# vsahni3/cross-attention-ViT

Measured on AMD Instinct MI355X. Metric: 3D patch-tokens/sec fwd+bwd, 2-modality 128^3 p16 ViT, higher is better.
Workload: dtype bf16; 1 GPU; configs[1]: ModelCross d=768 H=12 mlp=3072 2x2 blocks, 2 modalities, 128^3 volume, 16^3 patches (N=513), dropout 0; per_gpu_batch=126, global_batch=126, seq_len=513, parallelism=dp1, step=zero-grad + weight bf16 cast + fwd + loss + bwd, optimizer_step=excluded, launch=eager (one launch per kernel)

## Files before the change

cross-attention-vit_amd/csrc/gemm.hip:

```cpp
#include "xvit_common.h"

#include <atomic>
#include <algorithm>
#include <string>

namespace xvit {

struct GemmParams {
  const bf16* A = nullptr; const bf16* B = nullptr; void* C = nullptr; const float* bias = nullptr; const float* res = nullptr; bf16* aux = nullptr;
  int64_t lda = 0, ldb = 0, ldc = 0, ldr = 0, ldaux = 0;
  int64_t sA = 0, sB = 0, sC = 0, sBias = 0, sR = 0, sAux = 0;
  int M = 0, N = 0, K = 0, k_per_split = 0, split_k = 1, ntm = 0, ntn = 0;
  int c_f32 = 0, act = XVIT_ACT_NONE, accumulate = 0;
  int res_row_mod = 0, res_row_off = 0, seg_rows = 0, seg_skip = 0, row_off = 0;
  float* slab = nullptr;
  float* colsum = nullptr;
  float drop_p = 0.f, drop_inv = 1.f; uint64_t drop_seed = 0;
  const uint64_t* drop_epoch = nullptr;
  int aux_deriv = 0;
  int narrow_epi = 0;
  int ncg = 1;
  struct PatchGather {
    int mode = 0;
    int dp, hp, wp;
    int Dn, Wn;
    int Sy, Sz;
    int pcount, ntok, cls;
    int nb;
    int64_t sBt, sMd;
    uint32_t vol_bytes;
    uint32_t m_pcount, m_dn, m_wn, m_nb;
    uint32_t m_ntok;
  } g;
};

constexpr uint32_t GATHER_OOB = 0x80000000u;
constexpr uint32_t OOB = 0xFFFFFFF0u;
typedef __attribute__((__vector_size__(2 * sizeof(unsigned)))) unsigned u32x2_t;
// ... 234 lines not shown
      for (int kk = 0; kk < 2; ++kk) off[kk] = (uint32_t)(row * 128 + (((kk * 4 + (lane >> 4)) ^ swz_kc(row)) << 4));
    }
  }
  __device__ __forceinline__ bf16x8 read(const XVIT_LDS char* image, int t, int kk) const {
#ifdef XVIT_DEBUG_NO_LDSREAD
    if constexpr (W == 256) {
      u32x4_t v = {off[0] * 2654435761u, off[0] * 40503u + 12345u, (uint32_t)t * 0x9E3779B9u ^ off[0], 0x3F803F80u ^ (off[0] << 3)};
      v &= 0xBFFFBFFFu;
      asm volatile("" : "+v"(v));
      return __builtin_bit_cast(bf16x8, v);
    }
#endif
    if (KS) {
      const s16x4 lo = lds_read_tr16(image + off[t * 2 + 0] + kk * 32 * PITCH);
      const s16x4 hi = lds_read_tr16(image + off[t * 2 + 1] + kk * 32 * PITCH);
      s16x8 v = {lo[0], lo[1], lo[2], lo[3], hi[0], hi[1], hi[2], hi[3]};
      return __builtin_bit_cast(bf16x8, v);
    } else {
      return *(const XVIT_LDS bf16x8*)(image + off[kk] + t * 16 * 128);
    }
  }
};

template <bool A_KS, bool B_KS>
__global__ __launch_bounds__(256, 2) void gemm_kernel(const GemmParams p) {
  extern __shared__ __attribute__((aligned(16))) char smem_raw[];
  XVIT_LDS char* smem = (XVIT_LDS char*)smem_raw;
  const int tid = threadIdx.x, lane = tid & 63, wave = uniform(tid >> 6);
  const int wr = wave >> 1, wc = wave & 1;

  const int logical = xcd_logical(blockIdx.x, gridDim.x);
  const int tm = logical / p.ntn, tn = logical - tm * p.ntn;
  const int m0 = tm * BM, n0 = tn * BN;
  const int batch = blockIdx.z / p.split_k, split = blockIdx.z - batch * p.split_k;
  const int k_begin = split * p.k_per_split;
  const int k_end = min(p.K, k_begin + p.k_per_split);
  const int nk = (k_end - k_begin + BK - 1) / BK;
  TileLoader<A_KS, BM> la;
  TileLoader<B_KS, BN> lb;
  la.init(operand_tile<A_KS>(p.A + batch * p.sA, p.lda, m0, p.M, k_begin, k_end), p.lda, wave, lane);
  lb.init(operand_tile<B_KS>(p.B + batch * p.sB, p.ldb, n0, p.N, k_begin, k_end), p.ldb, wave, lane);
  TileFrag<A_KS, BM, 4> fa;
  TileFrag<B_KS, BN, 4> fb;
  fa.init(wr * 4, lane);
  fb.init(wc * 4, lane);

  f32x4 acc[4][4];
// ... 48 lines not shown
#pragma unroll
    for (int mi = 0; mi < 2; ++mi)
#pragma unroll
      for (int j = 0; j < 4; ++j)
#pragma unroll
        for (int r = 0; r < 4; ++r)
          slab[(mi * 16 + (lane >> 4) * 4 + r) * EPI_LD + j * 16 + (lane & 15)] = acc[pass * 2 + mi][j][r];
    const int row_base = m0 + wr * 64 + pass * 32;
#pragma unroll 1
    for (int it = 0; it < 8; ++it) {
      const int rl = it * 4 + (lane >> 4);
      const int row = row_base + rl;
      const f32x4 v = *(const XVIT_LDS f32x4*)(slab + rl * EPI_LD + (lane & 15) * 4);
      if (row < p.M && col < p.N) {
        if (part) {
          *(f32x4*)(part + (int64_t)row * p.N + col) = v;
        } else {
          cs4 += epilogue_apply_rt(p, v, row, col, cb, bias, res, aux);
        }
      }
    }
  }
  if (csum && !part) colsum_flush<16>(csum + col, cs4, col < p.N);
}

constexpr int TBM = 256, TBN = 256;
constexpr int T_OPER = TBM * BK * 2;
constexpr int T_STAGE = 2 * T_OPER;
constexpr int T_LDS = 2 * T_STAGE;

__device__ __forceinline__ uint32_t gather_soff_rows(const GemmParams::PatchGather& g, int ktg) { return 2u * gather_elem_off(g, ktg * 64); }
struct GatherStep { uint32_t a, b; };
__device__ __forceinline__ GatherStep gather_soff_wgrad(const GemmParams::PatchGather& g, int ktg, int64_t lda) {
  const int spk = g.pcount >> 6, smp = ktg / spk, r = ktg - smp * spk;
  const int wsteps = (g.Dn * g.Wn) >> 6, h = r / wsteps, wpart = (r - h * wsteps) * (64 / g.Dn);
  GatherStep o;
  o.a = (uint32_t)(((int64_t)smp * g.ntok + g.cls + r * 64) * lda * 2);
  o.b = 2u * (gather_sample_origin(g, smp) + (uint32_t)(h * g.hp * g.Sy + wpart * g.wp));
  return o;
}

template <int S, int PF, int NA, int NB>
__device__ __forceinline__ void mma_sched_steps() {
  constexpr int reads = (S + PF < 16 ? NA : 0) + (S >= 4 && S < 8 ? NB : 0);
  if constexpr (reads > 0) __builtin_amdgcn_sched_group_barrier(0x100, reads, 0);
  __builtin_amdgcn_sched_group_barrier(0x008, 4, 0);
// ... 381 lines not shown
  const int wl = pin_lane(lane);
  Transpose8 t;
  t.init(wl);
  ScatterEpi e;
  e.vol = (char*)p.C;
  const uint32_t col = (uint32_t)(col0 + (wl & 7) * 8);
  e.col_ok = col < (uint32_t)p.N;
  e.eoff = e.col_ok ? gather_elem_off(p.g, (int)col) : 0u;
  e.row = (uint32_t)(row0 + (wl >> 3));
  struct NoLoads {} none;
  transpose8_regions<0>(t, acc, smem + wave * EPI_WAVE_BYTES, none, [](NoLoads&) {}, [&](f32x4 v0, f32x4 v1, const NoLoads&, int) { scatter_body(p, e, v0, v1); });
}

#ifdef XVIT_GEMM_CLOCK_PROBE
__device__ long long xvit_dbg_clk[2 * 4096];
struct ClockProbe {
  long long c0, w0;
  __device__ ClockProbe() : c0(clock64()), w0(wall_clock64()) {}
  __device__ ~ClockProbe() {
    if (threadIdx.x == 0 && blockIdx.z == 0 && blockIdx.x < 4096) { xvit_dbg_clk[2 * blockIdx.x] = clock64() - c0; xvit_dbg_clk[2 * blockIdx.x + 1] = wall_clock64() - w0; }
  }
};
#endif
template <bool A_KS, bool B_KS, int WIDE_ACT, int GATHER = 0>
__global__ __launch_bounds__(512, 2) void gemm_big_kernel(const GemmParams p) {
  extern __shared__ __attribute__((aligned(16))) char smem_raw[];
  XVIT_LDS char* smem = (XVIT_LDS char*)smem_raw;
#ifdef XVIT_GEMM_CLOCK_PROBE
  ClockProbe clock_probe;
#endif
  const int tid = threadIdx.x, lane = tid & 63, wave = uniform(tid >> 6);
  const int wr = wave >> 2, wc = wave & 3;

  const int nblk = gridDim.x;
  const int logical = xcd_logical(blockIdx.x + nblk * blockIdx.z, nblk * gridDim.z);
  const int zz = logical / nblk, tile = logical - zz * nblk;
  const int grp = min(tile / (p.ntm * p.ncg), (p.ntn - 1) / p.ncg);
  const int rem = tile - grp * p.ntm * p.ncg;
  const int gw = min(p.ncg, p.ntn - grp * p.ncg);
  const int tm = rem / gw, tn = grp * p.ncg + (rem - tm * gw);
  const int m0 = tm * TBM, n0 = tn * TBN;
  const int batch = zz / p.split_k, split = zz - batch * p.split_k;
  const int k_begin = split * p.k_per_split;
  const int k_end = min(p.K, k_begin + p.k_per_split);
  const int nk = (k_end - k_begin + BK - 1) / BK;

  TileLoader<A_KS, TBM> la;
// ... 41 lines not shown
    uint32_t oa, ob;
    step_off(0, oa, ob);
    la.issue_at(smem, wave, oa);
    lb.issue_at(smem + T_OPER, wave, ob);
  }
  for (int kt = 0; kt < nk; ++kt) {
    asm volatile("s_waitcnt vmcnt(0)" ::: "memory");
    __syncthreads();
    const bool more = kt + 1 < nk;
    uint32_t soff_a, soff_b;
    step_off(kt + 1, soff_a, soff_b);
    XVIT_LDS char* nxt = smem + ((kt + 1) & 1) * T_STAGE;
    const XVIT_LDS char* sa = smem + (kt & 1) * T_STAGE;
    const XVIT_LDS char* sb = sa + T_OPER;
#ifndef XVIT_DEBUG_NO_MMA
    big_tile_mma<A_KS, B_KS>(sa, sb, fa, fb, acc, la, lb, more ? la.rsrc : null_rsrc, more ? lb.rsrc : null_rsrc, nxt, wave, soff_a, soff_b);
#endif
  }

  asm volatile("s_waitcnt vmcnt(0)" ::: "memory");
  __syncthreads();
  if constexpr (GATHER == 4) scatter_epilogue(p, acc, smem, wave, lane, m0 + wr * 128, n0 + wc * 64);
  else if constexpr (WIDE_ACT >= 0) wave_tile_epilogue_wide<WIDE_ACT>(p, acc, smem, wave, lane, m0 + wr * 128, n0 + wc * 64, batch);
  else wave_tile_epilogue<GATHER == 1>(p, acc, smem, wave, lane, m0 + wr * 128, n0 + wc * 64, batch, split);
}

__global__ void splitk_epilogue_kernel(const GemmParams p, int nbatch) {
  const int nv = p.N >> 2;
  const int64_t per = (int64_t)p.M * nv, total = per * nbatch;
  for (int64_t i = (int64_t)blockIdx.x * blockDim.x + threadIdx.x; i < total; i += (int64_t)gridDim.x * blockDim.x) {
    const int b = (int)(i / per);
    const int64_t r = i - (int64_t)b * per;
    const int row = (int)(r / nv), col = (int)(r - (int64_t)row * nv) * 4;
    f32x4 v = {0.f, 0.f, 0.f, 0.f};
    for (int s = 0; s < p.split_k; ++s) v += *(const f32x4*)(p.slab + (((int64_t)s * nbatch + b) * p.M + row) * p.N + col);
    const f32x4 o = epilogue_apply_rt(p, v, row, col, b * p.sC, p.bias ? p.bias + b * p.sBias : nullptr, p.res ? p.res + b * p.sR : nullptr,
                                      p.aux ? p.aux + b * p.sAux : nullptr);
    if (p.colsum) {
#pragma unroll
      for (int e = 0; e < 4; ++e) unsafeAtomicAdd(p.colsum + b * p.sBias + col + e, o[e]);
    }
  }
}

}

using namespace xvit;

static bool aligned16(const void* p) { return (reinterpret_cast<uintptr_t>(p) & 15) == 0; }

static std::atomic<int> g_gemm_tile{0};
static std::atomic<int> g_gemm_epi{0};
static std::atomic<int> g_gemm_group{0};

static bool use_big_tile(const xvit_gemm_args* a) {
  if (a->M < 256 || a->N < 256 || g_gemm_tile.load(std::memory_order_relaxed) == 1) return false;
  if (g_gemm_tile.load(std::memory_order_relaxed) == 2) return true;
  const int64_t big_blocks = (int64_t)((a->M + 255) / 256) * ((a->N + 255) / 256) * a->batch * (a->split_k > 0 ? a->split_k : 1);
  return big_blocks > 128;
}

static int k_per_split(int K, int split_k) {
  const int ktiles = (K + BK - 1) / BK;
  return ((ktiles + split_k - 1) / split_k) * BK;
}

static void set_tile_grid(GemmParams& p, int tile, int layout, bool grouped = true) {
  p.ntm = (p.M + tile - 1) / tile; p.ntn = (p.N + tile - 1) / tile;
  p.ncg = p.ntn;
  if (grouped) {
    const int forced = g_gemm_group.load(std::memory_order_relaxed);
    p.ncg = forced > 0 ? std::min(forced, p.ntn) : (layout == XVIT_GEMM_NT && p.ntn >= 6 ? 3 : p.ntn);
  }
}

template <bool A_KS, bool B_KS, int WIDE_ACT, int GATHER = 0>
static void launch_big(const GemmParams& p, int grid_z, hipStream_t s) {
  launch_lds<gemm_big_kernel<A_KS, B_KS, WIDE_ACT, GATHER>, T_LDS, 512>(dim3(p.ntm * p.ntn, 1, grid_z), s, p);
}
template <bool A_KS, bool B_KS>
static void launch_small(const GemmParams& p, int grid_z, hipStream_t s) {
  launch_lds<gemm_kernel<A_KS, B_KS>, GEMM_LDS, 256>(dim3(p.ntm * p.ntn, 1, grid_z), s, p);
}
static void launch_splitk_reduce(const GemmParams& p, int nbatch, hipStream_t s) {
  const int64_t work = (int64_t)nbatch * p.M * (p.N / 4);
  const int g = (int)((work + 255) / 256 > 4096 ? 4096 : (work + 255) / 256);
  hipLaunchKernelGGL(splitk_epilogue_kernel, dim3(g), dim3(256), 0, s, p, nbatch);
}

extern "C" int xvit_set_option(const char* name, int value) {
  XVIT_REQUIRE(name != nullptr, "xvit_set_option: null name");
  const std::string n(name);
  if (n == "gemm_tile") { XVIT_REQUIRE(value >= 0 && value <= 2, "xvit_set_option: gemm_tile must be 0 (auto), 1 (128x128 only) or 2 (256x256 whenever M, N >= 256)"); g_gemm_tile = value; return 0; }
  if (n == "gemm_group") { XVIT_REQUIRE(value >= 0 && value <= 4096, "xvit_set_option: gemm_group must be in [0, 4096]"); g_gemm_group = value; return 0; }
  if (n == "gemm_epilogue") { XVIT_REQUIRE(value == 0 || value == 1, "xvit_set_option: gemm_epilogue must be 0 (auto) or 1 (narrow)"); g_gemm_epi = value; return 0; }
  if (n == "attn_peel") { XVIT_REQUIRE(value >= 0 && value <= 2, "xvit_set_option: attn_peel must be 0 (token 0 stays on the tile grid), 1 (auto: large grids) or 2 (whenever N = 64 m + 1)"); set_attn_peel(value); return 0; }
  set_error("xvit_set_option: unknown option '%s'", name);
  return XVIT_ERR_ARG;
}

extern "C" int64_t xvit_gemm_workspace_bytes(const xvit_gemm_args* a) {
  if (!a || a->split_k <= 1) return 0;
  return (int64_t)a->split_k * a->batch * a->M * a->N * (int64_t)sizeof(float);
}

extern "C" int xvit_gemm(const xvit_gemm_args* a, xvit_stream_t stream) {
  XVIT_REQUIRE(a != nullptr, "xvit_gemm: null args");
  XVIT_REQUIRE(a->layout >= 0 && a->layout <= 2, "xvit_gemm: bad layout %d", a->layout);
  XVIT_REQUIRE(a->M > 0 && a->N > 0 && a->K > 0 && a->batch > 0, "xvit_gemm: M,N,K,batch must be > 0 (got %d,%d,%d,%d)", a->M, a->N, a->K, a->batch);
  XVIT_REQUIRE(a->A && a->B && a->C, "xvit_gemm: null A/B/C");
  const bool a_ks = a->layout == XVIT_GEMM_TN, b_ks = a->layout != XVIT_GEMM_NT;
  XVIT_REQUIRE(a_ks || a->K % 64 == 0, "xvit_gemm: K=%d must be a multiple of 64 when A is k-contiguous", a->K);
  XVIT_REQUIRE(b_ks || a->K % 64 == 0, "xvit_gemm: K=%d must be a multiple of 64 when B is k-contiguous", a->K);
  XVIT_REQUIRE(a->N % 4 == 0, "xvit_gemm: N=%d must be a multiple of 4 (use xvit_small_linear_*)", a->N);
  XVIT_REQUIRE(a->lda % 8 == 0 && a->ldb % 8 == 0 && a->stride_a % 8 == 0 && a->stride_b % 8 == 0, "xvit_gemm: lda/ldb/strides must be multiples of 8 elements");
  XVIT_REQUIRE(aligned16(a->A) && aligned16(a->B) && aligned16(a->C), "xvit_gemm: A/B/C must be 16-byte aligned");
  XVIT_REQUIRE(a->ldc % 4 == 0 && a->stride_c % 4 == 0, "xvit_gemm: ldc/stride_c must be multiples of 4");
  XVIT_REQUIRE(a->lda >= (a_ks ? a->M : a->K) && a->ldb >= (b_ks ? a->N : a->K) && a->ldc >= a->N, "xvit_gemm: leading dimension smaller than the row length");
  const int64_t a_rows = a_ks ? a->K : a->M, b_rows = b_ks ? a->K : a->N;
  XVIT_REQUIRE(a_rows * a->lda * 2 < (1ll << 31) && b_rows * a->ldb * 2 < (1ll << 31), "xvit_gemm: an operand matrix exceeds 2 GiB (unsupported addressing range)");
  XVIT_REQUIRE(a->split_k >= 1, "xvit_gemm: split_k must be >= 1");
  {
// ... 16 lines not shown
                 a->split_k, (long long)ws_need, (long long)a->workspace_bytes);

  GemmParams p;
  p.A = (const bf16*)a->A; p.B = (const bf16*)a->B; p.C = a->C; p.bias = a->bias; p.res = a->residual; p.aux = (bf16*)a->aux;
  p.lda = a->lda; p.ldb = a->ldb; p.ldc = a->ldc; p.ldr = a->ldr; p.ldaux = a->ldaux;
  p.sA = a->stride_a; p.sB = a->stride_b; p.sC = a->stride_c; p.sBias = a->stride_bias; p.sR = a->stride_r; p.sAux = a->stride_aux;
  p.M = a->M; p.N = a->N; p.K = a->K; p.split_k = a->split_k;
  p.k_per_split = k_per_split(a->K, a->split_k);
  p.c_f32 = a->c_dtype == XVIT_F32; p.act = a->act; p.accumulate = a->accumulate;
  p.res_row_mod = a->res_row_mod; p.res_row_off = a->res_row_off;
  p.seg_rows = a->out_seg_rows; p.seg_skip = a->out_seg_skip; p.row_off = a->out_row_off;
  p.slab = ws_need > 0 ? (float*)a->workspace : nullptr;
  p.colsum = a->colsum;
  XVIT_REQUIRE(a->dropout_p >= 0.f && a->dropout_p < 1.f, "xvit_gemm: dropout_p must be in [0, 1)");
  p.drop_p = a->dropout_p; p.drop_inv = 1.0f / (1.0f - a->dropout_p); p.drop_seed = a->dropout_seed;
  p.drop_epoch = a->dropout_p > 0.f ? drop_epoch_ptr() : nullptr;
  p.narrow_epi = g_gemm_epi.load(std::memory_order_relaxed);
  p.aux_deriv = a->aux_mode;
  hipStream_t s = (hipStream_t)stream;
  const int gz = a->batch * a->split_k;

  if (big) {
    set_tile_grid(p, TBM, a->layout);
    const bool wide = !p.c_f32 && !p.slab && !p.res && p.seg_rows == 0 && !p.narrow_epi && p.drop_p == 0.f && a->layout != XVIT_GEMM_TN &&
                      ((p.N | (int)p.ldc | (int)p.ldaux) & 7) == 0 && (a->layout == XVIT_GEMM_NT ? p.act != XVIT_ACT_DGELU : p.act != XVIT_ACT_GELU);
    if (wide && a->layout == XVIT_GEMM_NT && p.act == XVIT_ACT_NONE) launch_big<false, false, XVIT_ACT_NONE>(p, gz, s);
    else if (wide && a->layout == XVIT_GEMM_NT && p.aux_deriv) launch_big<false, false, ACT_GELU_D>(p, gz, s);
    else if (wide && a->layout == XVIT_GEMM_NT) launch_big<false, false, XVIT_ACT_GELU>(p, gz, s);
    else if (wide && p.act == XVIT_ACT_NONE) launch_big<false, true, XVIT_ACT_NONE>(p, gz, s);
    else if (wide && p.aux_deriv) launch_big<false, true, ACT_MULAUX>(p, gz, s);
    else if (wide) launch_big<false, true, XVIT_ACT_DGELU>(p, gz, s);
    else if (a->layout == XVIT_GEMM_NT) launch_big<false, false, -1>(p, gz, s);
    else if (a->layout == XVIT_GEMM_NN) launch_big<false, true, -1>(p, gz, s);
    else launch_big<true, true, -1>(p, gz, s);
  } else {
    set_tile_grid(p, BM, a->layout, false);
    switch (a->layout) {
      case XVIT_GEMM_NT: launch_small<false, false>(p, gz, s); break;
      case XVIT_GEMM_NN: launch_small<false, true>(p, gz, s); break;
      default: launch_small<true, true>(p, gz, s); break;
    }
  }
  if (p.slab) launch_splitk_reduce(p, a->batch, s);
  return check_launch("xvit_gemm");
}

static int64_t pe_rows(const xvit_patch_geom* g) {
  return (int64_t)g->M * g->B * (g->cls_rows + (int64_t)(g->D / g->dp) * (g->H / g->hp) * (g->W / g->wp));
}

static bool pe_geom_ok(const xvit_patch_geom* g) {
  if (!g || g->B <= 0 || g->M <= 0 || g->dp <= 0 || g->hp <= 0 || g->wp <= 0 || (g->cls_rows != 0 && g->cls_rows != 1)) return false;
  return !(g->D % g->dp || g->H % g->hp || g->W % g->wp);
}

extern "C" int xvit_patch_embed_supported(const xvit_patch_geom* g, int d) {
  if (!pe_geom_ok(g)) return 0;
  const int Dn = g->D / g->dp, Hn = g->H / g->hp, Wn = g->W / g->wp;
  const int64_t pd = (int64_t)g->dp * g->hp * g->wp, pcount = (int64_t)Dn * Hn * Wn;
  if (g->wp % 8 || 64 % g->wp || (g->hp * g->wp) % 64) return 0;
  if (pd % 256 || d % 256 || d < 256) return 0;
  const int64_t rows = pe_rows(g);
  if (rows < 2048) return 0;
  if ((int64_t)g->B * g->M * g->D * g->H * g->W * 2 >= (1ll << 31)) return 0;
  if (rows * d * 4 >= (1ll << 31) || pcount > (1 << 24)) return 0;
  return 1;
// ... 62 lines not shown
                                      int64_t workspace_bytes, xvit_stream_t stream) {
  XVIT_REQUIRE(img && g && dx && dW, "xvit_patch_embed_wgrad: null pointer");
  XVIT_REQUIRE(xvit_patch_embed_supported(g, d) == 1, "xvit_patch_embed_wgrad: geometry not supported by the fused kernel (xvit_patch_embed_supported)");
  const int64_t pd = (int64_t)g->dp * g->hp * g->wp;
  XVIT_REQUIRE(lddx >= d && lddx % 8 == 0 && lddw >= pd && lddw % 4 == 0, "xvit_patch_embed_wgrad: bad leading dimension");
  XVIT_REQUIRE(aligned16(img) && aligned16(dx) && aligned16(dW), "xvit_patch_embed_wgrad: pointers must be 16-byte aligned");
  XVIT_REQUIRE(pe_rows(g) * lddx * 2 < (1ll << 31), "xvit_patch_embed_wgrad: dx exceeds 2 GiB (unsupported addressing range)");
  const int64_t need = xvit_patch_embed_wgrad_workspace_bytes(g, d);
  XVIT_REQUIRE(need == 0 || (workspace && workspace_bytes >= need && aligned16(workspace)), "xvit_patch_embed_wgrad: needs %lld bytes of 16-byte aligned workspace (got %lld)",
               (long long)need, (long long)workspace_bytes);
  GemmParams p;
  pe_defaults(p);
  const bool aligned = pe_aligned(g);
  pe_fill(p, g, aligned ? 2 : 3);
  p.A = (const bf16*)dx; p.B = (const bf16*)img; p.C = dW;
  p.lda = lddx; p.ldc = lddw;
  p.M = d; p.N = (int)pd;
  p.K = (int)((int64_t)g->M * g->B * p.g.pcount);
  p.split_k = pe_wgrad_split(g, d);
  p.k_per_split = k_per_split(p.K, p.split_k);
  p.slab = need > 0 ? (float*)workspace : nullptr;
  set_tile_grid(p, TBM, XVIT_GEMM_TN, false);
  hipStream_t s = (hipStream_t)stream;
  if (aligned) launch_big<true, true, -1, 2>(p, p.split_k, s);
  else launch_big<true, true, -1, 3>(p, p.split_k, s);
  if (p.slab) launch_splitk_reduce(p, 1, s);
  return check_launch("xvit_patch_embed_wgrad");
}

extern "C" int xvit_patch_embed_dgrad_supported(const xvit_patch_geom* g, int d) {
  if (!pe_geom_ok(g)) return 0;
  if (g->wp % 8) return 0;
  if (d % 64 || d < 64) return 0;
  const int64_t rows = pe_rows(g);
  if (rows < 2048) return 0;
  if ((int64_t)g->B * g->M * g->D * g->H * g->W >= (1ll << 30)) return 0;
  if (rows * d * 2 >= (1ll << 31)) return 0;
  if ((int64_t)(g->D / g->dp) * (g->H / g->hp) * (g->W / g->wp) > (1 << 24)) return 0;
  return 1;
}

extern "C" int xvit_patch_embed_dgrad(const void* dx, int64_t lddx, const void* W, int64_t ldw, const xvit_patch_geom* g, int d, void* dimg, int dimg_dtype,
                                      xvit_stream_t stream) {
  XVIT_REQUIRE(dx && W && g && dimg, "xvit_patch_embed_dgrad: null pointer");
  XVIT_REQUIRE(dimg_dtype == XVIT_F32 || dimg_dtype == XVIT_BF16, "xvit_patch_embed_dgrad: bad output dtype %d", dimg_dtype);
  XVIT_REQUIRE(xvit_patch_embed_dgrad_supported(g, d) == 1, "xvit_patch_embed_dgrad: geometry not supported by the fused kernel (xvit_patch_embed_dgrad_supported)");
  const int64_t pd = (int64_t)g->dp * g->hp * g->wp;
  XVIT_REQUIRE(lddx >= d && lddx % 8 == 0 && ldw >= pd && ldw % 8 == 0, "xvit_patch_embed_dgrad: bad leading dimension");
  XVIT_REQUIRE(aligned16(dx) && aligned16(W) && aligned16(dimg), "xvit_patch_embed_dgrad: pointers must be 16-byte aligned");
// ... 18 lines not shown
```

cross-attention-vit_amd/csrc/linear_f32.hip:

```cpp
#include "xvit_common.h"

namespace xvit {

struct F32Params {
  const float* A; const float* W; float* C; const float* bias; const float* res; float* slab;
  bf16* c_bf16; bf16* z_bf16;
  int64_t lda, ldw, ldc, ldr, ldcb, ldzb;
  int M, N, K, k_per_split, split_k, act;
  Dropout drop;
};

__device__ __forceinline__ void f32_epilogue(const F32Params& p, float v, int row, int col) {
  if (p.bias) v += p.bias[col];
  if (p.act == XVIT_ACT_GELU) {
    if (p.z_bf16) p.z_bf16[(int64_t)row * p.ldzb + col] = f2bf(v);
    v = gelu_f(v);
  }
  if (p.drop.on()) v = p.drop.at_run_time().keep((uint64_t)row * p.N + col) ? v * p.drop.inv : 0.f;
  if (p.res) v += p.res[(int64_t)row * p.ldr + col];
  p.C[(int64_t)row * p.ldc + col] = v;
  if (p.c_bf16) p.c_bf16[(int64_t)row * p.ldcb + col] = f2bf(v);
}

__global__ __launch_bounds__(64) void linear_f32_kernel(const F32Params p) {
  const int lane = threadIdx.x, r = lane & 31, h = lane >> 5;
  const int ntn = (p.N + 31) >> 5;
  const int tm = blockIdx.x / ntn, tn = blockIdx.x - tm * ntn, split = blockIdx.y;
  const int m0 = tm * 32, n0 = tn * 32;
  const int kb = split * p.k_per_split, ke = min(p.K, kb + p.k_per_split);
  const float* ap = p.A + (int64_t)min(m0 + r, p.M - 1) * p.lda + 4 * h;
  const float* wp = p.W + (int64_t)min(n0 + r, p.N - 1) * p.ldw + 4 * h;
  f32x16 acc;
#pragma unroll
  for (int i = 0; i < 16; ++i) acc[i] = 0.f;
#pragma unroll 2
  for (int k = kb; k < ke; k += 16) {
    const f32x4 a0 = *(const f32x4*)(ap + k), a1 = *(const f32x4*)(ap + k + 8);
    const f32x4 w0 = *(const f32x4*)(wp + k), w1 = *(const f32x4*)(wp + k + 8);
#pragma unroll
    for (int e = 0; e < 4; ++e) acc = __builtin_amdgcn_mfma_f32_32x32x2f32(a0[e], w0[e], acc, 0, 0, 0);
#pragma unroll
    for (int e = 0; e < 4; ++e) acc = __builtin_amdgcn_mfma_f32_32x32x2f32(a1[e], w1[e], acc, 0, 0, 0);
  }
  const int col = n0 + r;
  if (col >= p.N) return;
#pragma unroll
  for (int t = 0; t < 16; ++t) {
    const int row = m0 + acc_row(t, h);
    if (row < p.M) {
      if (p.slab) p.slab[((int64_t)split * p.M + row) * p.N + col] = acc[t];
      else f32_epilogue(p, acc[t], row, col);
    }
  }
}

__global__ void linear_f32_reduce_kernel(const F32Params p) {
  const int64_t total = (int64_t)p.M * p.N;
  for (int64_t i = (int64_t)blockIdx.x * blockDim.x + threadIdx.x; i < total; i += (int64_t)gridDim.x * blockDim.x) {
    const int row = (int)(i / p.N), col = (int)(i - (int64_t)row * p.N);
    float v = 0.f;
    for (int s = 0; s < p.split_k; ++s) v += p.slab[(int64_t)s * total + i];
    f32_epilogue(p, v, row, col);
  }
}

static int f32_split(int M, int N, int K) {
  const int tiles = ((M + 31) / 32) * ((N + 31) / 32);
  int split = 1024 / (tiles > 0 ? tiles : 1);
  const int max_split = K / 64;
  if (split > max_split) split = max_split;
  if (split > 32) split = 32;
  return split < 1 ? 1 : split;
}

}

using namespace xvit;

extern "C" int64_t xvit_linear_f32_workspace_bytes(int M, int N, int K) {
  if (M <= 0 || N <= 0 || K <= 0) return 0;
  const int split = f32_split(M, N, K);
  return split > 1 ? (int64_t)split * M * N * (int64_t)sizeof(float) : 0;
}

extern "C" int xvit_linear_f32(const float* x, int64_t ldx, const float* W, int64_t ldw, const float* bias, float* y, int64_t ldy, int M, int N, int K,
                               int act, void* z_bf16, int64_t ldz, const float* residual, int64_t ldr, void* y_bf16, int64_t ldyb, float dropout_p,
                               uint64_t dropout_seed, void* workspace, int64_t workspace_bytes, xvit_stream_t stream) {
  XVIT_REQUIRE(x && W && y, "xvit_linear_f32: null x/W/y");
  XVIT_REQUIRE(M > 0 && N > 0 && K > 0 && K % 16 == 0, "xvit_linear_f32: need M, N > 0 and K a positive multiple of 16 (got %d, %d, %d)", M, N, K);
  XVIT_REQUIRE(ldx % 4 == 0 && ldw % 4 == 0 && ldx >= K && ldw >= K && ldy >= N, "xvit_linear_f32: ldx/ldw must be multiples of 4 and >= K, ldy >= N");
  XVIT_REQUIRE(((uintptr_t)x & 15) == 0 && ((uintptr_t)W & 15) == 0, "xvit_linear_f32: x and W must be 16-byte aligned");
  XVIT_REQUIRE(act == XVIT_ACT_NONE || act == XVIT_ACT_GELU, "xvit_linear_f32: act must be NONE or GELU");
  XVIT_REQUIRE(dropout_p >= 0.f && dropout_p < 1.f, "xvit_linear_f32: dropout_p must be in [0, 1)");
  XVIT_REQUIRE(!residual || ldr >= N, "xvit_linear_f32: ldr < N");
  XVIT_REQUIRE((!z_bf16 || ldz >= N) && (!y_bf16 || ldyb >= N), "xvit_linear_f32: ldz / ldyb < N");
  F32Params p;
  p.A = x; p.W = W; p.C = y; p.bias = bias; p.res = residual; p.c_bf16 = (bf16*)y_bf16; p.z_bf16 = (bf16*)z_bf16;
  p.lda = ldx; p.ldw = ldw; p.ldc = ldy; p.ldr = ldr; p.ldcb = ldyb; p.ldzb = ldz;
  p.M = M; p.N = N; p.K = K; p.act = act;
  p.split_k = f32_split(M, N, K);
  p.k_per_split = (((K + 15) / 16 + p.split_k - 1) / p.split_k) * 16;
  p.drop = Dropout(dropout_p, dropout_seed);
  const int64_t need = xvit_linear_f32_workspace_bytes(M, N, K);
  XVIT_REQUIRE(need == 0 || (workspace && workspace_bytes >= need), "xvit_linear_f32: needs %lld bytes of workspace (got %lld)", (long long)need,
               (long long)workspace_bytes);
  p.slab = need > 0 ? (float*)workspace : nullptr;
  hipStream_t s = (hipStream_t)stream;
  const dim3 grid(((M + 31) / 32) * ((N + 31) / 32), p.split_k);
  hipLaunchKernelGGL(linear_f32_kernel, grid, dim3(64), 0, s, p);
  if (p.slab) hipLaunchKernelGGL(linear_f32_reduce_kernel, dim3(grid_for((int64_t)M * N, 256, 2048)), dim3(256), 0, s, p);
  return check_launch("xvit_linear_f32");
}
```

cross-attention-vit_amd/csrc/xvit_common.h:

```cpp
#pragma once
#include <hip/hip_runtime.h>
#include <stdint.h>

#include <mutex>
#include <type_traits>

#include "../../include/xvit.h"

namespace xvit {

typedef __bf16 bf16;
typedef __attribute__((ext_vector_type(8))) __bf16 bf16x8;
typedef __attribute__((ext_vector_type(4))) __bf16 bf16x4;
typedef __attribute__((ext_vector_type(2))) __bf16 bf16x2;
typedef __attribute__((ext_vector_type(4))) short s16x4;
typedef __attribute__((ext_vector_type(8))) short s16x8;
typedef __attribute__((ext_vector_type(4))) float f32x4;
typedef __attribute__((ext_vector_type(16))) float f32x16;
typedef __attribute__((ext_vector_type(2))) float f32x2;

#define XVIT_LDS __attribute__((address_space(3)))

constexpr int kWave = 64;

void set_error(const char* fmt, ...);
int check_launch(const char* what);
const uint64_t* drop_epoch_ptr();
void set_attn_peel(int v);

template <auto KERNEL, int LDS, int BLOCK, class... Args>
static void launch_lds(dim3 grid, hipStream_t s, Args... args) {
  static const hipError_t opt_in = hipFuncSetAttribute((const void*)KERNEL, hipFuncAttributeMaxDynamicSharedMemorySize, LDS);
  (void)opt_in;
  hipLaunchKernelGGL(KERNEL, grid, dim3(BLOCK), LDS, s, args...);
}

template <auto KERNEL, class... Args>
static hipError_t launch_dyn_lds(dim3 grid, dim3 block, size_t lds, hipStream_t s, Args... args) {
  static std::mutex lock;
  static size_t limit = 64 * 1024;
  {
    std::lock_guard<std::mutex> hold(lock);
    if (lds > limit) {
      const hipError_t e = hipFuncSetAttribute((const void*)KERNEL, hipFuncAttributeMaxDynamicSharedMemorySize, (int)lds);
      if (e != hipSuccess) return e;
      limit = lds;
    }
  }
  hipLaunchKernelGGL(KERNEL, grid, block, lds, s, args...);
  return hipSuccess;
}
// ... 9 lines not shown
  if (dtype == XVIT_F32) f(float{});
  else f(bf16{});
}

#define XVIT_REQUIRE(cond, ...)            \
  do {                                     \
    if (!(cond)) {                         \
      ::xvit::set_error(__VA_ARGS__);      \
      return XVIT_ERR_ARG;                 \
    }                                      \
  } while (0)

__device__ __forceinline__ float bf2f(bf16 v) { return (float)v; }
__device__ __forceinline__ bf16 f2bf(float v) { return (bf16)v; }

__device__ __forceinline__ bf16x4 to_bf16x4(const f32x4& a) { return bf16x4{f2bf(a[0]), f2bf(a[1]), f2bf(a[2]), f2bf(a[3])}; }
__device__ __forceinline__ bf16x8 to_bf16x8(const f32x4& a, const f32x4& b) {
  return bf16x8{f2bf(a[0]), f2bf(a[1]), f2bf(a[2]), f2bf(a[3]), f2bf(b[0]), f2bf(b[1]), f2bf(b[2]), f2bf(b[3])};
}

__device__ __forceinline__ int lane_id() { return threadIdx.x & 63; }

__device__ __forceinline__ int uniform(int v) { return __builtin_amdgcn_readfirstlane(v); }

__device__ __forceinline__ __amdgpu_buffer_rsrc_t make_rsrc(const void* base, uint32_t bytes) {
  return __builtin_amdgcn_make_buffer_rsrc(const_cast<void*>(base), 0, bytes, 0x00020000);
}

__device__ __forceinline__ uint32_t clamp_bytes(int64_t b) {
  return b <= 0 ? 0u : (b > 0x7FFFFFFFll ? 0x7FFFFFFFu : (uint32_t)b);
}

#ifndef XVIT_GLDS_POLICY
#define XVIT_GLDS_POLICY ""
#endif
__device__ __forceinline__ void glds16(__amdgpu_buffer_rsrc_t r, XVIT_LDS void* lds_base, uint32_t voff, uint32_t soff) {
  const uint32_t m0v = (uint32_t)(uintptr_t)lds_base;
  asm volatile("s_mov_b32 m0, %3\n\ts_nop 0\n\tbuffer_load_dwordx4 %0, %1, %2 offen" XVIT_GLDS_POLICY " lds"
               :
               : "v"(voff), "s"(r), "s"(soff), "s"(m0v)
               : "memory");
}
__device__ __forceinline__ void glds4(__amdgpu_buffer_rsrc_t r, XVIT_LDS void* lds_base, uint32_t voff, uint32_t soff) {
  const uint32_t m0v = (uint32_t)(uintptr_t)lds_base;
  asm volatile("s_mov_b32 m0, %3\n\ts_nop 0\n\tbuffer_load_dword %0, %1, %2 offen lds"
               :
// ... 147 lines not shown
```

cross-attention-vit_amd/xvit/_lib.py:

```python
from __future__ import annotations

import ctypes as C
import os

_HERE = os.path.dirname(os.path.abspath(__file__))
LIB_PATH = os.environ.get("XVIT_LIB") or os.path.join(_HERE, "libxvit_hip.so")

i32, i64, f32, u64, vp = C.c_int32, C.c_int64, C.c_float, C.c_uint64, C.c_void_p


class GemmArgs(C.Structure):
    _fields_ = [(n, i32) for n in (
        "layout", "M", "N", "K", "batch", "c_dtype", "act", "accumulate", "split_k",
        "res_row_mod", "res_row_off", "out_seg_rows", "out_seg_skip", "out_row_off", "aux_mode")] + [
        (n, vp) for n in ("A", "B", "C", "bias", "residual", "aux")] + [
        (n, i64) for n in ("lda", "ldb", "ldc", "ldr", "ldaux",
                           "stride_a", "stride_b", "stride_c", "stride_bias", "stride_r", "stride_aux")] + [
        ("workspace", vp), ("workspace_bytes", i64), ("colsum", vp), ("dropout_p", f32), ("reserved2", i32), ("dropout_seed", u64)]


class PatchGeom(C.Structure):
    _fields_ = [(n, i32) for n in ("B", "M", "D", "H", "W", "dp", "hp", "wp", "cls_rows")]


# ... 56 lines not shown
    "xvit_cast_f32_bf16": [vp, vp, i64, vp],
    "xvit_add_cast_f32_bf16": [vp, vp, vp, vp, i64, vp],
    "xvit_rows_combine": [vp, i32, i64, vp, i32, i64, vp, i32, i64, vp, i32, i64, i32, i32, vp],
    "xvit_colsum": [vp, i32, i64, vp, i32, i32, i32, vp, i64, vp],
    "xvit_dropout": [vp, vp, i32, i64, f32, u64, vp],
    "xvit_cu_trace": [vp, i32, i32, vp],
    "xvit_binary_metrics_step": [vp, i64, vp, i32, i32, vp, vp],
    "xvit_mean_ce": [vp, vp, f32, vp, vp, vp, i32, i32, i32, vp],
    "xvit_resize_pad_crop_i16": [vp, vp, i32, i32, i32, i32, i32, i32, i32, f32, vp],
    "xvit_augment_draw": [C.POINTER(AugmentConfig), vp, i32, i32, i32, i32, i32, i32, i32, i32, u64, vp, i32, vp],
    "xvit_augment_apply": [vp, i32, vp, i32, vp, i32, i32, i32, i32, i32, i32, i32, f32, vp],
    "xvit_volume_stats": [vp, i32, i32, i64, C.POINTER(NormConfig), vp, vp, vp, i64, vp],
    "xvit_set_option": [C.c_char_p, i32],
    "xvit_set_dropout_epoch": [C.c_void_p],
    "xvit_adam_step": [vp, vp, i32, f32, f32, f32, f32, f32, i32, f32, vp],
    "xvit_grad_sqnorm_partials": [vp, vp, i32, vp, vp],
    "xvit_adam_prologue": [vp, i32, vp, f32, f32, f32, i32, vp],
    "xvit_adam_step_dev": [vp, vp, i32, vp, f32, f32, f32, f32, vp],
    "xvit_grad_pack_bf16": [C.POINTER(GradSegment), i32, vp, i64, f32, vp],
    "xvit_grad_unpack_bf16": [vp, vp, i64, f32, vp],
}
EXPORTS = sorted(list(SIGNATURES) + ["xvit_version", "xvit_last_error_string", "xvit_gemm_workspace_bytes", "xvit_linear_f32_workspace_bytes",
                                    "xvit_colsum_workspace_bytes", "xvit_layernorm_bwd_workspace_bytes", "xvit_patch_embed_wgrad_workspace_bytes", "xvit_attn_fp8_workspace_bytes",
                                    "xvit_attn_fwd_workspace_bytes", "xvit_attn_bwd_workspace_bytes", "xvit_volume_stats_workspace_bytes"])

_lib = None


def load() -> C.CDLL:
    global _lib
    if _lib is None:
        if not os.path.exists(LIB_PATH):
            raise RuntimeError(
                f"xvit: {LIB_PATH} is missing. Build it with `python cross-attention-vit_amd/build.py` "
                "(hipcc, gfx950). There is no CPU or PyTorch fallback for this path.")
        lib = C.CDLL(LIB_PATH)
        for name, argtypes in SIGNATURES.items():
            fn = getattr(lib, name)
            fn.argtypes = argtypes
            fn.restype = C.c_int
        lib.xvit_gemm_workspace_bytes.argtypes = [C.POINTER(GemmArgs)]
        lib.xvit_gemm_workspace_bytes.restype = C.c_int64
        lib.xvit_linear_f32_workspace_bytes.argtypes = [i32, i32, i32]
        lib.xvit_linear_f32_workspace_bytes.restype = C.c_int64
        for name in ("xvit_colsum_workspace_bytes", "xvit_layernorm_bwd_workspace_bytes"):
            getattr(lib, name).argtypes = [i32, i32]
            getattr(lib, name).restype = C.c_int64
        lib.xvit_attn_fp8_workspace_bytes.argtypes = [i32, i32, i32, i32]
        lib.xvit_attn_fp8_workspace_bytes.restype = C.c_int64
        for name in ("xvit_attn_fwd_workspace_bytes", "xvit_attn_bwd_workspace_bytes"):
            getattr(lib, name).argtypes = [i32, i32, i32]
            getattr(lib, name).restype = C.c_int64
        lib.xvit_patch_embed_wgrad_workspace_bytes.argtypes = [C.POINTER(PatchGeom), i32]
        lib.xvit_patch_embed_wgrad_workspace_bytes.restype = C.c_int64
        lib.xvit_volume_stats_workspace_bytes.argtypes = [i32]
        lib.xvit_volume_stats_workspace_bytes.restype = C.c_int64
        lib.xvit_version.restype = C.c_int
        lib.xvit_last_error_string.restype = C.c_char_p
        _lib = lib
    return _lib


def check(rc: int, what: str) -> None:
    if rc != 0:
        msg = load().xvit_last_error_string().decode(errors="replace")
        raise RuntimeError(f"{what} failed (rc={rc}): {msg}")
```

cross-attention-vit_amd/xvit/ops.py:

```python
from __future__ import annotations

import ctypes as C
import os

import torch

from . import _lib
from ._lib import GemmArgs

BF16, F32 = 0, 1
NT, NN, TN = 0, 1, 2
ACT_NONE, ACT_GELU, ACT_DGELU = 0, 1, 2


_cur_dev = torch._C._cuda_getDevice
_raw_stream = torch._C._cuda_getCurrentRawStream


def _stream() -> int:
    return _raw_stream(_cur_dev())


PROFILE = None
DETERMINISTIC = os.environ.get("XVIT_DETERMINISTIC", "0") == "1"


def set_deterministic(on: bool = True):
    global DETERMINISTIC
    DETERMINISTIC = bool(on)


GEMM_TILE = 0


def set_option(name: str, value: int):
    global GEMM_TILE
    _lib.check(_lib.load().xvit_set_option(name.encode(), int(value)), "xvit_set_option")
    if name == "gemm_tile":
        GEMM_TILE = int(value)


_DROP_EPOCH = None


def set_dropout_epoch(counter):
    global _DROP_EPOCH
    if counter is not None and not (counter.is_cuda and counter.dtype == torch.int64 and counter.numel() == 1):
        raise RuntimeError("set_dropout_epoch: need a one-element int64 GPU tensor (or None)")
    _lib.check(_lib.load().xvit_set_dropout_epoch(counter.data_ptr() if counter is not None else None), "xvit_set_dropout_epoch")
    _DROP_EPOCH = counter


PROFILE_SHAPES = False


def _run(name, work, kind, rc_fn, what):
    if PROFILE is None:
        _lib.check(rc_fn(), what)
        return
    s, e = torch.cuda.Event(enable_timing=True), torch.cuda.Event(enable_timing=True)
    s.record()
    _lib.check(rc_fn(), what)
# ... 643 lines not shown
```

include/xvit.h:

```cpp
#ifndef XVIT_H
#define XVIT_H

#include <stdint.h>

#ifdef __cplusplus
extern "C" {
#endif

#define XVIT_VERSION 310

enum { XVIT_OK = 0, XVIT_ERR_ARG = -1, XVIT_ERR_UNSUPPORTED = -2 };
enum { XVIT_BF16 = 0, XVIT_F32 = 1, XVIT_I16 = 2  };

typedef void* xvit_stream_t;

int xvit_version(void);
const char* xvit_last_error_string(void);
int xvit_set_option(const char* name, int value);
int xvit_set_dropout_epoch(const uint64_t* device_counter);

enum { XVIT_GEMM_NT = 0, XVIT_GEMM_NN = 1, XVIT_GEMM_TN = 2 };
enum { XVIT_ACT_NONE = 0,
       XVIT_ACT_GELU = 1,
       XVIT_ACT_DGELU = 2   };
enum { XVIT_ACC_STORE = 0, XVIT_ACC_ADD = 1  };

typedef struct xvit_gemm_args {
  int32_t layout, M, N, K, batch;
  int32_t c_dtype;
  int32_t act;
  int32_t accumulate;
  int32_t split_k;
  int32_t res_row_mod, res_row_off;
  int32_t out_seg_rows, out_seg_skip, out_row_off;
  int32_t aux_mode;
  const void* A; const void* B; void* C;
  const float* bias;
  const float* residual;
  void* aux;
  int64_t lda, ldb, ldc, ldr, ldaux;
  int64_t stride_a, stride_b, stride_c, stride_bias, stride_r, stride_aux;
// ... 176 lines not shown
```

Before: 3.731 million patch-tokens/s.

## Fuse split-K reduction into GEMM via last-arriver tickets

Split-K GEMMs (bf16 small/big tiles, patch-embed wgrad, f32 linear) now take a per-tile atomic ticket after writing partials. The last-arriving split reduces the slab and applies the epilogue in place, so the separate reduce kernel launch is skipped. Tickets live in a static device array keyed by device, stream and capture. This removes a launch and a full pass over the slab, but the reduce for each tile now runs serially on one workgroup, with extra fences, atomics and a new kernel variant.

```diff
diff --git a/cross-attention-vit_amd/csrc/gemm.hip b/cross-attention-vit_amd/csrc/gemm.hip
--- a/cross-attention-vit_amd/csrc/gemm.hip
+++ b/cross-attention-vit_amd/csrc/gemm.hip
@@ -14,6 +14,7 @@
   int c_f32 = 0, act = XVIT_ACT_NONE, accumulate = 0;
   int res_row_mod = 0, res_row_off = 0, seg_rows = 0, seg_skip = 0, row_off = 0;
   float* slab = nullptr;
+  unsigned* tickets = nullptr;
   float* colsum = nullptr;
   float drop_p = 0.f, drop_inv = 1.f; uint64_t drop_seed = 0;
   const uint64_t* drop_epoch = nullptr;
@@ -294,7 +295,26 @@
   }
 };
 
-template <bool A_KS, bool B_KS>
+__device__ __forceinline__ void splitk_reduce_at(const GemmParams& p, int nbatch, int b, int row, int col) {
+  f32x4 v = {0.f, 0.f, 0.f, 0.f};
+  for (int s = 0; s < p.split_k; ++s) v += *(const f32x4*)(p.slab + (((int64_t)s * nbatch + b) * p.M + row) * p.N + col);
+  const f32x4 o = epilogue_apply_rt(p, v, row, col, b * p.sC, p.bias ? p.bias + b * p.sBias : nullptr, p.res ? p.res + b * p.sR : nullptr,
+                                    p.aux ? p.aux + b * p.sAux : nullptr);
+  if (p.colsum) {
+#pragma unroll
+    for (int e = 0; e < 4; ++e) unsafeAtomicAdd(p.colsum + b * p.sBias + col + e, o[e]);
+  }
+}
+__device__ __forceinline__ void splitk_reduce_range(const GemmParams& p, int nbatch, int b, int row0, int row1, int col0, int col1, int64_t t, int64_t nthr) {
+  const int nv = (col1 - col0) >> 2;
+  const int64_t total = (int64_t)(row1 - row0) * nv;
+  for (int64_t i = t; i < total; i += nthr) {
+    const int r = (int)(i / nv);
+    splitk_reduce_at(p, nbatch, b, row0 + r, col0 + (int)(i - (int64_t)r * nv) * 4);
+  }
+}
+
+template <bool A_KS, bool B_KS, bool FUSED = false>
 __global__ __launch_bounds__(256, 2) void gemm_kernel(const GemmParams p) {
   extern __shared__ __attribute__((aligned(16))) char smem_raw[];
   XVIT_LDS char* smem = (XVIT_LDS char*)smem_raw;
@@ -389,6 +409,10 @@
     }
   }
   if (csum && !part) colsum_flush<16>(csum + col, cs4, col < p.N);
+  if constexpr (FUSED) {
+    if (splitk_last_arriver(p.tickets + batch * gridDim.x + logical, p.split_k, (XVIT_LDS int*)smem))
+      splitk_reduce_range(p, nbatch, batch, m0, min(m0 + BM, p.M), n0, min(n0 + BN, p.N), tid, 256);
+  }
 }
 
 constexpr int TBM = 256, TBN = 256;
@@ -816,7 +840,7 @@
   }
 };
 #endif
-template <bool A_KS, bool B_KS, int WIDE_ACT, int GATHER = 0>
+template <bool A_KS, bool B_KS, int WIDE_ACT, int GATHER = 0, bool FUSED = false>
 __global__ __launch_bounds__(512, 2) void gemm_big_kernel(const GemmParams p) {
   extern __shared__ __attribute__((aligned(16))) char smem_raw[];
   XVIT_LDS char* smem = (XVIT_LDS char*)smem_raw;
@@ -904,7 +928,13 @@
   __syncthreads();
   if constexpr (GATHER == 4) scatter_epilogue(p, acc, smem, wave, lane, m0 + wr * 128, n0 + wc * 64);
   else if constexpr (WIDE_ACT >= 0) wave_tile_epilogue_wide<WIDE_ACT>(p, acc, smem, wave, lane, m0 + wr * 128, n0 + wc * 64, batch);
-  else wave_tile_epilogue<GATHER == 1>(p, acc, smem, wave, lane, m0 + wr * 128, n0 + wc * 64, batch, split);
+  else {
+    wave_tile_epilogue<GATHER == 1>(p, acc, smem, wave, lane, m0 + wr * 128, n0 + wc * 64, batch, split);
+    if constexpr (FUSED) {
+      if (splitk_last_arriver(p.tickets + batch * nblk + tile, p.split_k, (XVIT_LDS int*)smem))
+        splitk_reduce_range(p, gridDim.z / p.split_k, batch, m0, min(m0 + TBM, p.M), n0, min(n0 + TBN, p.N), tid, 512);
+    }
+  }
 }
 
 __global__ void splitk_epilogue_kernel(const GemmParams p, int nbatch) {
@@ -913,15 +943,8 @@
   for (int64_t i = (int64_t)blockIdx.x * blockDim.x + threadIdx.x; i < total; i += (int64_t)gridDim.x * blockDim.x) {
     const int b = (int)(i / per);
     const int64_t r = i - (int64_t)b * per;
-    const int row = (int)(r / nv), col = (int)(r - (int64_t)row * nv) * 4;
-    f32x4 v = {0.f, 0.f, 0.f, 0.f};
-    for (int s = 0; s < p.split_k; ++s) v += *(const f32x4*)(p.slab + (((int64_t)s * nbatch + b) * p.M + row) * p.N + col);
-    const f32x4 o = epilogue_apply_rt(p, v, row, col, b * p.sC, p.bias ? p.bias + b * p.sBias : nullptr, p.res ? p.res + b * p.sR : nullptr,
-                                      p.aux ? p.aux + b * p.sAux : nullptr);
-    if (p.colsum) {
-#pragma unroll
-      for (int e = 0; e < 4; ++e) unsafeAtomicAdd(p.colsum + b * p.sBias + col + e, o[e]);
-    }
+    const int row = (int)(r / nv);
+    splitk_reduce_at(p, nbatch, b, row, (int)(r - (int64_t)row * nv) * 4);
   }
 }
 
@@ -934,6 +957,55 @@
 static std::atomic<int> g_gemm_tile{0};
 static std::atomic<int> g_gemm_epi{0};
 static std::atomic<int> g_gemm_group{0};
+
+static std::atomic<int> g_splitk_fused{1};
+static std::atomic<long long> g_splitk_fallbacks{0};
+namespace xvit {
+constexpr int kSplitkSlots = 512;
+__device__ unsigned xvit_splitk_tickets[kSplitkSlots * kSplitkSlot];
+
+static bool splitk_fused_pays(int producer, int split_k) {
+  (void)producer; (void)split_k;
+  return true;
+}
+
+struct SplitkSlotKey {
+  int device; hipStream_t stream; unsigned long long capture;
+  bool operator==(const SplitkSlotKey& o) const { return device == o.device && stream == o.stream && capture == o.capture; }
+};
+
+unsigned* splitk_ticket_slot(hipStream_t s, int64_t tickets, int producer, int split_k) {
+  const int mode = g_splitk_fused.load(std::memory_order_relaxed);
+  if (mode == 0 || (mode != 3 && !splitk_fused_pays(producer, split_k))) return nullptr;
+  if (tickets > kSplitkSlot || mode == 2) { g_splitk_fallbacks.fetch_add(1, std::memory_order_relaxed); return nullptr; }
+  static std::mutex lock;
+  static SplitkSlotKey keys[kSplitkSlots];
+  static int used = 0;
+  static unsigned* base[64] = {};
+  SplitkSlotKey k{0, s, 0ull};
+  hipStreamCaptureStatus status = hipStreamCaptureStatusNone;
+  if (hipGetDevice(&k.device) != hipSuccess || k.device < 0 || k.device >= 64 || hipStreamGetCaptureInfo(s, &status, &k.capture) != hipSuccess) {
+    (void)hipGetLastError();
+    g_splitk_fallbacks.fetch_add(1, std::memory_order_relaxed);
+    return nullptr;
+  }
+  if (status != hipStreamCaptureStatusActive) k.capture = 0ull;
+  std::lock_guard<std::mutex> hold(lock);
+  if (!base[k.device] && hipGetSymbolAddress((void**)&base[k.device], HIP_SYMBOL(xvit_splitk_tickets)) != hipSuccess) {
+    (void)hipGetLastError();
+    base[k.device] = nullptr;
+    g_splitk_fallbacks.fetch_add(1, std::memory_order_relaxed);
+    return nullptr;
+  }
+  int slot = 0;
+  while (slot < used && !(keys[slot] == k)) ++slot;
+  if (slot == used) {
+    if (used == kSplitkSlots) { g_splitk_fallbacks.fetch_add(1, std::memory_order_relaxed); return nullptr; }
+    keys[used++] = k;
+  }
+  return base[k.device] + (int64_t)slot * kSplitkSlot;
+}
+}
 
 static bool use_big_tile(const xvit_gemm_args* a) {
   if (a->M < 256 || a->N < 256 || g_gemm_tile.load(std::memory_order_relaxed) == 1) return false;
@@ -958,10 +1030,14 @@
 
 template <bool A_KS, bool B_KS, int WIDE_ACT, int GATHER = 0>
 static void launch_big(const GemmParams& p, int grid_z, hipStream_t s) {
+  if constexpr (WIDE_ACT < 0 && GATHER != 1 && GATHER != 4) {
+    if (p.slab && p.tickets) return launch_lds<gemm_big_kernel<A_KS, B_KS, WIDE_ACT, GATHER, true>, T_LDS, 512>(dim3(p.ntm * p.ntn, 1, grid_z), s, p);
+  }
   launch_lds<gemm_big_kernel<A_KS, B_KS, WIDE_ACT, GATHER>, T_LDS, 512>(dim3(p.ntm * p.ntn, 1, grid_z), s, p);
 }
 template <bool A_KS, bool B_KS>
 static void launch_small(const GemmParams& p, int grid_z, hipStream_t s) {
+  if (p.slab && p.tickets) return launch_lds<gemm_kernel<A_KS, B_KS, true>, GEMM_LDS, 256>(dim3(p.ntm * p.ntn, 1, grid_z), s, p);
   launch_lds<gemm_kernel<A_KS, B_KS>, GEMM_LDS, 256>(dim3(p.ntm * p.ntn, 1, grid_z), s, p);
 }
 static void launch_splitk_reduce(const GemmParams& p, int nbatch, hipStream_t s) {
@@ -976,10 +1052,13 @@
   if (n == "gemm_tile") { XVIT_REQUIRE(value >= 0 && value <= 2, "xvit_set_option: gemm_tile must be 0 (auto), 1 (128x128 only) or 2 (256x256 whenever M, N >= 256)"); g_gemm_tile = value; return 0; }
   if (n == "gemm_group") { XVIT_REQUIRE(value >= 0 && value <= 4096, "xvit_set_option: gemm_group must be in [0, 4096]"); g_gemm_group = value; return 0; }
   if (n == "gemm_epilogue") { XVIT_REQUIRE(value == 0 || value == 1, "xvit_set_option: gemm_epilogue must be 0 (auto) or 1 (narrow)"); g_gemm_epi = value; return 0; }
+  if (n == "splitk_fused") { XVIT_REQUIRE(value >= 0 && value <= 3, "xvit_set_option: splitk_fused must be 0 (reduce kernel), 1 (fused, default), 2 (ticket pool reported exhausted) or 3 (fused ignoring the measured gates)"); g_splitk_fused = value; return 0; }
   if (n == "attn_peel") { XVIT_REQUIRE(value >= 0 && value <= 2, "xvit_set_option: attn_peel must be 0 (token 0 stays on the tile grid), 1 (auto: large grids) or 2 (whenever N = 64 m + 1)"); set_attn_peel(value); return 0; }
   set_error("xvit_set_option: unknown option '%s'", name);
   return XVIT_ERR_ARG;
 }
+
+extern "C" int64_t xvit_splitk_fused_fallbacks(void) { return g_splitk_fallbacks.load(std::memory_order_relaxed); }
 
 extern "C" int64_t xvit_gemm_workspace_bytes(const xvit_gemm_args* a) {
   if (!a || a->split_k <= 1) return 0;
@@ -1042,6 +1121,7 @@
 
   if (big) {
     set_tile_grid(p, TBM, a->layout);
+    if (p.slab) p.tickets = splitk_ticket_slot(s, (int64_t)a->batch * p.ntm * p.ntn, kSplitkBig, p.split_k);
     const bool wide = !p.c_f32 && !p.slab && !p.res && p.seg_rows == 0 && !p.narrow_epi && p.drop_p == 0.f && a->layout != XVIT_GEMM_TN &&
                       ((p.N | (int)p.ldc | (int)p.ldaux) & 7) == 0 && (a->layout == XVIT_GEMM_NT ? p.act != XVIT_ACT_DGELU : p.act != XVIT_ACT_GELU);
     if (wide && a->layout == XVIT_GEMM_NT && p.act == XVIT_ACT_NONE) launch_big<false, false, XVIT_ACT_NONE>(p, gz, s);
@@ -1055,13 +1135,14 @@
     else launch_big<true, true, -1>(p, gz, s);
   } else {
     set_tile_grid(p, BM, a->layout, false);
+    if (p.slab) p.tickets = splitk_ticket_slot(s, (int64_t)a->batch * p.ntm * p.ntn, kSplitkSmall, p.split_k);
     switch (a->layout) {
       case XVIT_GEMM_NT: launch_small<false, false>(p, gz, s); break;
       case XVIT_GEMM_NN: launch_small<false, true>(p, gz, s); break;
       default: launch_small<true, true>(p, gz, s); break;
     }
   }
-  if (p.slab) launch_splitk_reduce(p, a->batch, s);
+  if (p.slab && !p.tickets) launch_splitk_reduce(p, a->batch, s);
   return check_launch("xvit_gemm");
 }
 
@@ -1170,9 +1251,10 @@
   p.slab = need > 0 ? (float*)workspace : nullptr;
   set_tile_grid(p, TBM, XVIT_GEMM_TN, false);
   hipStream_t s = (hipStream_t)stream;
+  if (p.slab) p.tickets = splitk_ticket_slot(s, (int64_t)p.ntm * p.ntn, kSplitkBig, p.split_k);
   if (aligned) launch_big<true, true, -1, 2>(p, p.split_k, s);
   else launch_big<true, true, -1, 3>(p, p.split_k, s);
-  if (p.slab) launch_splitk_reduce(p, 1, s);
+  if (p.slab && !p.tickets) launch_splitk_reduce(p, 1, s);
   return check_launch("xvit_patch_embed_wgrad");
 }
 
diff --git a/cross-attention-vit_amd/csrc/linear_f32.hip b/cross-attention-vit_amd/csrc/linear_f32.hip
--- a/cross-attention-vit_amd/csrc/linear_f32.hip
+++ b/cross-attention-vit_amd/csrc/linear_f32.hip
@@ -4,6 +4,7 @@
 
 struct F32Params {
   const float* A; const float* W; float* C; const float* bias; const float* res; float* slab;
+  unsigned* tickets;
   bf16* c_bf16; bf16* z_bf16;
   int64_t lda, ldw, ldc, ldr, ldcb, ldzb;
   int M, N, K, k_per_split, split_k, act;
@@ -22,6 +23,14 @@
   if (p.c_bf16) p.c_bf16[(int64_t)row * p.ldcb + col] = f2bf(v);
 }
 
+__device__ __forceinline__ void f32_reduce_at(const F32Params& p, int row, int col) {
+  const int64_t total = (int64_t)p.M * p.N, i = (int64_t)row * p.N + col;
+  float v = 0.f;
+  for (int s = 0; s < p.split_k; ++s) v += p.slab[(int64_t)s * total + i];
+  f32_epilogue(p, v, row, col);
+}
+
+template <bool FUSED>
 __global__ __launch_bounds__(64) void linear_f32_kernel(const F32Params p) {
   const int lane = threadIdx.x, r = lane & 31, h = lane >> 5;
   const int ntn = (p.N + 31) >> 5;
@@ -43,13 +52,20 @@
     for (int e = 0; e < 4; ++e) acc = __builtin_amdgcn_mfma_f32_32x32x2f32(a1[e], w1[e], acc, 0, 0, 0);
   }
   const int col = n0 + r;
-  if (col >= p.N) return;
+  if (col < p.N) {
 #pragma unroll
-  for (int t = 0; t < 16; ++t) {
-    const int row = m0 + acc_row(t, h);
-    if (row < p.M) {
-      if (p.slab) p.slab[((int64_t)split * p.M + row) * p.N + col] = acc[t];
-      else f32_epilogue(p, acc[t], row, col);
+    for (int t = 0; t < 16; ++t) {
+      const int row = m0 + acc_row(t, h);
+      if (row < p.M) {
+        if (p.slab) p.slab[((int64_t)split * p.M + row) * p.N + col] = acc[t];
+        else f32_epilogue(p, acc[t], row, col);
+      }
+    }
+  }
+  if constexpr (FUSED) {
+    if (splitk_last_arriver(p.tickets + blockIdx.x, p.split_k, nullptr) && col < p.N) {
+      const int rows = min(32, p.M - m0);
+      for (int rr = h; rr < rows; rr += 2) f32_reduce_at(p, m0 + rr, col);
     }
   }
 }
@@ -57,10 +73,8 @@
 __global__ void linear_f32_reduce_kernel(const F32Params p) {
   const int64_t total = (int64_t)p.M * p.N;
   for (int64_t i = (int64_t)blockIdx.x * blockDim.x + threadIdx.x; i < total; i += (int64_t)gridDim.x * blockDim.x) {
-    const int row = (int)(i / p.N), col = (int)(i - (int64_t)row * p.N);
-    float v = 0.f;
-    for (int s = 0; s < p.split_k; ++s) v += p.slab[(int64_t)s * total + i];
-    f32_epilogue(p, v, row, col);
+    const int row = (int)(i / p.N);
+    f32_reduce_at(p, row, (int)(i - (int64_t)row * p.N));
   }
 }
 
@@ -107,7 +121,9 @@
   p.slab = need > 0 ? (float*)workspace : nullptr;
   hipStream_t s = (hipStream_t)stream;
   const dim3 grid(((M + 31) / 32) * ((N + 31) / 32), p.split_k);
-  hipLaunchKernelGGL(linear_f32_kernel, grid, dim3(64), 0, s, p);
-  if (p.slab) hipLaunchKernelGGL(linear_f32_reduce_kernel, dim3(grid_for((int64_t)M * N, 256, 2048)), dim3(256), 0, s, p);
+  p.tickets = p.slab ? splitk_ticket_slot(s, grid.x, kSplitkF32, p.split_k) : nullptr;
+  if (p.tickets) hipLaunchKernelGGL(linear_f32_kernel<true>, grid, dim3(64), 0, s, p);
+  else hipLaunchKernelGGL(linear_f32_kernel<false>, grid, dim3(64), 0, s, p);
+  if (p.slab && !p.tickets) hipLaunchKernelGGL(linear_f32_reduce_kernel, dim3(grid_for((int64_t)M * N, 256, 2048)), dim3(256), 0, s, p);
   return check_launch("xvit_linear_f32");
 }
diff --git a/cross-attention-vit_amd/csrc/xvit_common.h b/cross-attention-vit_amd/csrc/xvit_common.h
--- a/cross-attention-vit_amd/csrc/xvit_common.h
+++ b/cross-attention-vit_amd/csrc/xvit_common.h
@@ -27,6 +27,10 @@
 int check_launch(const char* what);
 const uint64_t* drop_epoch_ptr();
 void set_attn_peel(int v);
+
+constexpr int kSplitkSlot = 1024;
+enum { kSplitkBig = 0, kSplitkSmall = 1, kSplitkF32 = 2 };
+unsigned* splitk_ticket_slot(hipStream_t s, int64_t tickets, int producer, int split_k);
 
 template <auto KERNEL, int LDS, int BLOCK, class... Args>
 static void launch_lds(dim3 grid, hipStream_t s, Args... args) {
@@ -82,6 +86,30 @@
 __device__ __forceinline__ int lane_id() { return threadIdx.x & 63; }
 
 __device__ __forceinline__ int uniform(int v) { return __builtin_amdgcn_readfirstlane(v); }
+
+__device__ __forceinline__ bool splitk_last_arriver(unsigned* ticket, int split_k, XVIT_LDS int* flag) {
+  asm volatile("s_waitcnt vmcnt(0)" ::: "memory");
+  if (flag) __syncthreads();
+  int last = 0;
+  if (threadIdx.x == 0) {
+    __builtin_amdgcn_fence(__ATOMIC_RELEASE, "agent");
+    asm volatile("s_waitcnt vmcnt(0)" ::: "memory");
+    last = __hip_atomic_fetch_add(ticket, 1u, __ATOMIC_RELAXED, __HIP_MEMORY_SCOPE_AGENT) == (unsigned)(split_k - 1);
+    if (last) {
+      __hip_atomic_store(ticket, 0u, __ATOMIC_RELAXED, __HIP_MEMORY_SCOPE_AGENT);
+      __builtin_amdgcn_fence(__ATOMIC_ACQUIRE, "agent");
+      asm volatile("s_waitcnt vmcnt(0)" ::: "memory");
+    }
+    if (flag) *flag = last;
+  }
+  if (flag) {
+    __syncthreads();
+    last = *flag;
+  } else {
+    last = __builtin_amdgcn_readfirstlane(last);
+  }
+  return last != 0;
+}
 
 __device__ __forceinline__ __amdgpu_buffer_rsrc_t make_rsrc(const void* base, uint32_t bytes) {
   return __builtin_amdgcn_make_buffer_rsrc(const_cast<void*>(base), 0, bytes, 0x00020000);
diff --git a/cross-attention-vit_amd/xvit/_lib.py b/cross-attention-vit_amd/xvit/_lib.py
--- a/cross-attention-vit_amd/xvit/_lib.py
+++ b/cross-attention-vit_amd/xvit/_lib.py
@@ -102,7 +102,7 @@
 }
 EXPORTS = sorted(list(SIGNATURES) + ["xvit_version", "xvit_last_error_string", "xvit_gemm_workspace_bytes", "xvit_linear_f32_workspace_bytes",
                                     "xvit_colsum_workspace_bytes", "xvit_layernorm_bwd_workspace_bytes", "xvit_patch_embed_wgrad_workspace_bytes", "xvit_attn_fp8_workspace_bytes",
-                                    "xvit_attn_fwd_workspace_bytes", "xvit_attn_bwd_workspace_bytes", "xvit_volume_stats_workspace_bytes"])
+                                    "xvit_attn_fwd_workspace_bytes", "xvit_attn_bwd_workspace_bytes", "xvit_volume_stats_workspace_bytes", "xvit_splitk_fused_fallbacks"])
 
 _lib = None
 
@@ -135,6 +135,8 @@
         lib.xvit_patch_embed_wgrad_workspace_bytes.restype = C.c_int64
         lib.xvit_volume_stats_workspace_bytes.argtypes = [i32]
         lib.xvit_volume_stats_workspace_bytes.restype = C.c_int64
+        lib.xvit_splitk_fused_fallbacks.argtypes = []
+        lib.xvit_splitk_fused_fallbacks.restype = C.c_int64
         lib.xvit_version.restype = C.c_int
         lib.xvit_last_error_string.restype = C.c_char_p
         _lib = lib
diff --git a/cross-attention-vit_amd/xvit/ops.py b/cross-attention-vit_amd/xvit/ops.py
--- a/cross-attention-vit_amd/xvit/ops.py
+++ b/cross-attention-vit_amd/xvit/ops.py
@@ -38,6 +38,10 @@
     _lib.check(_lib.load().xvit_set_option(name.encode(), int(value)), "xvit_set_option")
     if name == "gemm_tile":
         GEMM_TILE = int(value)
+
+
+def splitk_fused_fallbacks() -> int:
+    return int(_lib.load().xvit_splitk_fused_fallbacks())
 
 
 _DROP_EPOCH = None
diff --git a/include/xvit.h b/include/xvit.h
--- a/include/xvit.h
+++ b/include/xvit.h
@@ -7,7 +7,7 @@
 extern "C" {
 #endif
 
-#define XVIT_VERSION 310
+#define XVIT_VERSION 311
 
 enum { XVIT_OK = 0, XVIT_ERR_ARG = -1, XVIT_ERR_UNSUPPORTED = -2 };
 enum { XVIT_BF16 = 0, XVIT_F32 = 1, XVIT_I16 = 2  };
@@ -17,6 +17,7 @@
 int xvit_version(void);
 const char* xvit_last_error_string(void);
 int xvit_set_option(const char* name, int value);
+int64_t xvit_splitk_fused_fallbacks(void);
 int xvit_set_dropout_epoch(const uint64_t* device_counter);
 
 enum { XVIT_GEMM_NT = 0, XVIT_GEMM_NN = 1, XVIT_GEMM_TN = 2 };
```

Result: slower. 3.445 million patch-tokens/s (-7.7%).
